# DeJhon-Huang/TrueTrace-Unity-Pathtracer

Hardware: AMD Instinct MI355X
Metric: Mrays/sec (primary+1-bounce) on Sponza CWBVH at 1080p; % HBM roofline (higher is better)
Workload: dtype f32

## Files before the change

### truetrace-unity-pathtracer_amd/csrc/tt_trace.hip

```cpp
#include "tt_launch.h"
#include "tt_wide.h"

#ifndef TT_LEAF_REFILL_MIN
#define TT_LEAF_REFILL_MIN (TT_LEAF_POOL ? 16 : TT_REFILL_MIN)
#endif

namespace {
template <int INFO, int LEAF = 0>
__device__ __forceinline__ bool write_record(const TraceArgs& A, uint32_t ray_index, uint32_t pix, float col_w,
                                             const Best& best, const LaneRay& wr, int32_t inst_mesh = 0,
                                             int32_t inst_tri_offset = 0) {
    tt_ray_data* R = A.rays + ray_index;
    const int32_t best_mesh = LEAF ? (best.tri_id != -1 ? inst_mesh : 0) : best.mesh_id;
    auto tri_offset_of_best = [&]() -> int32_t {
        if (LEAF) return best.tri_id != -1 ? inst_tri_offset : A.mesh[0].TriOffset;
        return A.mesh[best.mesh_id].TriOffset;
    };
    if (INFO != 0) {
        if (pix < A.n_pixels) {
            uint4 o;
            bool write = false;
            if (INFO == 1) {
                const int32_t to = tri_offset_of_best();
                o = make_uint4((uint32_t)best_mesh, (uint32_t)(best.tri_id - to),
                               __float_as_uint(best.u), __float_as_uint(best.v));
                write = true;
            } else {
                const float w = col_w;
                if (w == -1.0f || (float)A.bounce == w) {
                    write = true;
                    const bool miss = best.t == A.far_plane;
                    if ((A.flags & TT_TRACE_USE_RESTIRGI) && !miss) {
                        const int32_t to = tri_offset_of_best();
                        o.x = (uint32_t)best_mesh;
                        o.y = (uint32_t)(best.tri_id - to);
                        o.z = (uint32_t)(best.u * 65535.0f) | ((uint32_t)(best.v * 65535.0f) << 16);
                    } else {
                        LaneRay w = wr;
                        if (LEAF == 1) {
                            const uint4* rp = reinterpret_cast<const uint4*>(R);
                            const uint4 r0 = rp[0], r1 = rp[1];
                            w.ox = __uint_as_float(r0.x);
                            w.oy = __uint_as_float(r0.y);
                            w.oz = __uint_as_float(r0.z);
                            w.dx = __uint_as_float(r1.x);
                            w.dy = __uint_as_float(r1.y);
                            w.dz = __uint_as_float(r1.z);
                        }
                        if ((A.flags & TT_TRACE_USE_ASVGF) || !miss) {
                            o.x = __float_as_uint(w.dx);
                            o.y = __float_as_uint(w.dy);
                            o.z = __float_as_uint(w.dz);
                        } else {
                            o.x = __float_as_uint(w.dx * best.t + w.ox);
                            o.y = __float_as_uint(w.dy * best.t + w.oy);
                            o.z = __float_as_uint(w.dz * best.t + w.oz);
                        }
                    }
                    o.w = miss ? 1u : 0u;
                }
            }
            if (write) reinterpret_cast<uint4*>(A.info)[pix] = o;
        }
    }
    const uint32_t uv = (uint32_t)(best.u * 65535.0f) | ((uint32_t)(best.v * 65535.0f) << 16);
    const uint4 hit = make_uint4((uint32_t)best_mesh, (uint32_t)best.tri_id, __float_as_uint(best.t), uv);
    reinterpret_cast<uint4*>(R)[2] = hit;
    if (A.hits_out) {
        const u32x4 v = {hit.x, hit.y, hit.z, hit.w};
        __builtin_amdgcn_raw_buffer_store_b128(v, buffer_rsrc(A.hits_out, 0x7fffffff), (ray_index - A.ray_offset) << 4,
                                               0, 0);
    }
    return best.t != A.far_plane;
}

__device__ __forceinline__ void keep_record(const TraceArgs& A, uint32_t ray_index) {
    if (A.hits_out) {
        const uint4 h = reinterpret_cast<const uint4*>(A.rays + ray_index)[2];
        const u32x4 v = {h.x, h.y, h.z, h.w};
        __builtin_amdgcn_raw_buffer_store_b128(v, buffer_rsrc(A.hits_out, 0x7fffffff), (ray_index - A.ray_offset) << 4,
                                               0, 0);
    }
}

static_assert(TT_CHUNK_BIG == 64, "the adaptive order maps one dequeue (TT_CHUNK_BIG rays) to one 64-ray chunk");
#ifndef TT_ORDER_MIN_REPS
#define TT_ORDER_MIN_REPS 32
#endif
__device__ __forceinline__ void record_chunk_cost(const TraceArgs& A, bool swizzle, uint32_t ray_index, int32_t reps) {
    if (reps < TT_ORDER_MIN_REPS) return;
    const uint32_t local = ray_index - A.ray_offset;
    uint32_t c = local >> 6;
    if (swizzle) {
        const uint32_t py = fastdiv(local, A.div_width), px = local - py * A.width;
        c = (py >> 3) * (A.width >> 3) + (px >> 3);
    }
    atomicMax(A.chunk_cost + c, (uint32_t)reps);
}
}


namespace {
__device__ __forceinline__ bool root_leaf_hit(const RootLeaf& R, const LaneRay& r, float max_distance) {
    const float adjx = __uint_as_float(rl_byte(R.e, 0) << 23) * r.ix;
    const float adjy = __uint_as_float(rl_byte(R.e, 1) << 23) * r.iy;
    const float adjz = __uint_as_float(rl_byte(R.e, 2) << 23) * r.iz;
    const float orgx = r.ix * (R.px - r.ox);
    const float orgy = r.iy * (R.py - r.oy);
    const float orgz = r.iz * (R.pz - r.oz);
    const bool nx = r.dx < 0.0f, ny = r.dy < 0.0f, nz = r.dz < 0.0f;
    const uint32_t x_min = rl_byte(nx ? R.qhi : R.qlo, 0), x_max = rl_byte(nx ? R.qlo : R.qhi, 0);
    const uint32_t y_min = rl_byte(ny ? R.qhi : R.qlo, 1), y_max = rl_byte(ny ? R.qlo : R.qhi, 1);
    const uint32_t z_min = rl_byte(nz ? R.qhi : R.qlo, 2), z_max = rl_byte(nz ? R.qlo : R.qhi, 2);
    const float tminx = fma_((float)x_min, adjx, orgx);
    const float tminy = fma_((float)y_min, adjy, orgy);
    const float tminz = fma_((float)z_min, adjz, orgz);
    const float tmaxx = fma_((float)x_max, adjx, orgx);
    const float tmaxy = fma_((float)y_max, adjy, orgy);
    const float tmaxz = fma_((float)z_max, adjz, orgz);
    const float tmin = fmaxf(fmaxf(tminx, tminy), fmaxf(tminz, 1e-8f));
    float tmaxz_c;
    asm("v_min_f32 %0, %1, %2" : "=v"(tmaxz_c) : "v"(tmaxz), "v"(max_distance));
    const float tmax = fminf(fminf(tmaxx, tmaxy), tmaxz_c);
    return tmin < tmax;
}
}


template <bool STATS, bool MATCHECK, int INFO, bool IND, bool ORD, int LEAF = 0>
__device__ __forceinline__ void trace_body(const TraceArgs& A) {
    static_assert(!LEAF || (!STATS && !MATCHECK && !ORD), "the leaf-TLAS form has no stats / material / order variants");
    constexpr bool POOL = LEAF != 0 && TT_LEAF_POOL != 0;
    constexpr int tt_lds_depth = lds_depth_of<LEAF>();
    static_assert(!POOL || TT_CHUNK_BIG == TT_WAVE, "the prepared-ray pool holds one chunk, one slot per lane");
    __shared__ uint2 s_stack[tt_lds_depth][TT_BLOCK];
    __shared__ uint4 s_pool[POOL ? 3 : 1][TT_BLOCK];
    (void)s_pool;
    LeafEntry L{};
    if (LEAF) L = load_leaf_mesh<true>(A.leaf, A.root.base_tri + firstbithigh(A.root.bits));
    const uint32_t tid = threadIdx.x;
    zero_next_control(A.ctl_next, tid);
    const uint32_t gtid = blockIdx.x * TT_BLOCK + tid;
    const uint32_t spill_stride = gridDim.x * TT_BLOCK;
    uint2* __restrict__ spill = A.spill;
    (void)gtid;
    (void)spill_stride;
    (void)spill;
    const uint32_t lane = tid & (TT_WAVE - 1);
#ifdef TT_DIAG_BLOCKS
    if (tid < TT_DB_N) tt_db[tid] = 0ull;
    __syncthreads();
#endif

    uint32_t pool_next = 0, pool_end = 0, more = 1;
    const uint32_t wave_id = blockIdx.x * (TT_BLOCK / TT_WAVE) + (tid >> 6);
    SegState S{blockIdx.x % TT_SEGS, 0u, 0u};
    const uint32_t n_rays = IND ? launch_ray_count(A) : A.n_rays;
    const uint32_t n_tiles = (n_rays + 63u) >> 6;
    const bool swizzle = IND ? (A.tile_swizzle && n_rays == A.n_pixels) : (A.tile_swizzle != 0u);
    const __amdgpu_buffer_rsrc_t nodes = buffer_rsrc(A.nodes, A.n_nodes * (uint32_t)TT_NODE_STRIDE);
    const __amdgpu_buffer_rsrc_t tris = buffer_rsrc(A.tris, A.n_tris * (uint32_t)sizeof(TriPos));

    constexpr uint32_t TT_IDLE = 0x80000000u;
    uint32_t ray_index = 0;
    uint32_t pix = 0;
    float col_w = 0.0f;
    bool pending = false;
    LaneRay ray{}, wray{};
    Best best{};
    uint2 cg = make_uint2(0u, 0u), tg = make_uint2(0u, TT_IDLE);
    uint32_t oct = 0;
    int32_t stack_size = 0, tlas_ss = -1;
    int32_t NodeOffset = 0, TriOffset = 0, MatOffset = 0, mesh_id = -1, Reps = 0;
    if (LEAF) {
        NodeOffset = L.off.y;
        TriOffset = L.off.x;
        MatOffset = L.off.z;
        mesh_id = L.mesh_id;
    }
    uint32_t c_nodes = 0, c_tris = 0, c_blas = 0, c_acc = 0, c_rays = 0, c_hits = 0, c_reps = 0, c_ovf = 0;
    uint32_t d_iter = 0, d_node_lanes = 0, d_node_iters = 0, d_tri_lanes = 0, d_tri_iters = 0, d_active_lanes = 0;
    uint32_t d_lead_same = 0, d_uniform = 0;
    auto world_ray = [&]() -> LaneRay { return wray; };
    auto ray_of = [&](uint32_t widx) -> uint32_t {
        uint32_t local = widx;
        if (swizzle) {
            const uint32_t tw = A.width >> 3;
            const uint32_t t = widx >> 6, l = widx & 63u;
            const uint32_t ty = fastdiv(t, A.div_tiles), tx = t - ty * tw;
            local = (ty * 8u + (l >> 3)) * A.width + tx * 8u + (l & 7u);
        }
        return A.ray_offset + local;
    };
    (void)ray_of;

#if TT_ROOT_LEAF
    const bool rl_ok = A.root.ok != 0u;
#endif
    auto enter_blas = [&]() {
            TT_DB(8);
            const uint32_t mo = firstbithigh(tg.y);
            tg.y &= ~(1u << mo);
            const LeafEntry e = load_leaf_mesh<true>(A.leaf, tg.x + mo);
            mesh_id = e.mesh_id;
            NodeOffset = e.off.y;
            TriOffset = e.off.x;
            bool ok = true;
            if (tg.y != 0u) TT_PUSH(tg, ok);
            if (ok && (cg.y & 0xff000000u)) TT_PUSH(cg, ok);
            tg.y = 0u;
            if (ok) {
                tlas_ss = stack_size;
                MatOffset = e.off.z;
                enter_object_space(e, ray, oct, cg);
                if (STATS) c_blas++;
            } else {
                tg.y = TT_IDLE;
                if (STATS) c_ovf++;
                TT_REPORT_OVERFLOW(A);
                keep_record(A, ray_index);
            }
    };
    auto finish_ray = [&]() {
        const bool hit = write_record<INFO, LEAF>(A, ray_index, pix, col_w, best, world_ray(), mesh_id, TriOffset);
        if (STATS) c_hits += hit ? 1u : 0u;
        (void)hit;
        if (ORD) record_chunk_cost(A, swizzle, ray_index, Reps);
    };
    constexpr uint32_t REFILL_MIN = LEAF ? TT_LEAF_REFILL_MIN : TT_REFILL_MIN;
    while (true) {
        TT_DB(0);
        const uint64_t idle = __ballot((int32_t)tg.y < 0);
        const uint32_t n_idle = (uint32_t)__builtin_popcount((uint32_t)idle) + (uint32_t)__builtin_popcount((uint32_t)(idle >> 32));
        const bool pool_dry = !more && pool_next >= pool_end;
#if TT_DRAIN_PRIO
        if (pool_dry) __builtin_amdgcn_s_setprio(TT_DRAIN_PRIO);
#endif
        const bool to_wide = TT_WIDE && pool_dry && n_idle < TT_WAVE && TT_WAVE - n_idle <= TT_WIDE_ENTER;
        if ((n_idle == TT_WAVE && pool_dry) || (n_idle >= REFILL_MIN && !pool_dry) || to_wide) {
            if (pending) {
                TT_DB(1);
                finish_ray();
                pending = false;
            }
        }
        if (n_idle == TT_WAVE && pool_dry) break;
#if TT_WIDE
        if (to_wide) {
            TT_DB(13);
            WideState st{{ray, world_ray(), cg, tg, oct, stack_size, tlas_ss, NodeOffset, TriOffset, MatOffset, Reps,
                          ray_index, tid, gtid, (int32_t)tg.y >= 0},
                         best, mesh_id, pix, col_w};
            regroup<2, LEAF>(st, __ballot((int32_t)tg.y >= 0), lane);
            auto finish_wide = [&](const WideState& w) {
                const bool hit = write_record<INFO, LEAF>(A, w.ray_index, w.pix, w.col_w, w.best, w.wray, mesh_id, TriOffset);
                if (STATS) c_hits += hit ? 1u : 0u;
                if (ORD) record_chunk_cost(A, swizzle, w.ray_index, w.Reps);
            };
            auto exhaust_wide = [&](const WideState& w) {
                keep_record(A, w.ray_index);
                if (ORD) record_chunk_cost(A, swizzle, w.ray_index, w.Reps);
            };
            wide_phase<STATS, MATCHECK, 2, LEAF>(A, st, s_stack, spill, spill_stride, nodes, tris, lane,
                                           Counters{c_nodes, c_tris, c_blas, c_acc, c_hits, c_reps, c_ovf},
                                           finish_wide, exhaust_wide);
            break;
        }
#endif
        if (n_idle >= REFILL_MIN && !pool_dry) {
            TT_DB(2);
#if TT_LONG_PRIO
            if (__ballot((int32_t)tg.y >= 0 && Reps >= TT_LONG_PRIO) != 0ull) __builtin_amdgcn_s_setprio(TT_LONG_PRIO_LEVEL);
            else __builtin_amdgcn_s_setprio(0);
#endif
            const uint32_t avail = pool_end - pool_next;
            uint32_t new_base = 0, new_count = 0;
            if (avail < n_idle && more) {
                new_count = sched_reserve(A.ctl, n_rays, n_tiles, lane, n_idle - avail, wave_id, S, new_base);
                more = new_count > 0 ? 1u : 0u;
                if (ORD && A.order && new_count > 0)
                    new_base = (__builtin_amdgcn_readfirstlane(A.order[new_base >> 6]) << 6) | (new_base & 63u);
            }
            const PoolTake pt = pool_take<TT_UNIFORM_POOL != 0>(idle, n_idle, new_base, new_count, pool_next, pool_end, more);
            const uint32_t widx = pt.widx;
            pool_next = pt.pool_next;
            pool_end = pt.pool_end;
            more = pt.more;
            if constexpr (POOL) {
                const uint32_t pcol = tid - lane;
                const bool take = (int32_t)tg.y < 0 && widx != 0xffffffffu;
                const bool take_left = take && lane_prefix(idle) < min(avail, n_idle);
                uint4 p0 = make_uint4(0u, 0u, 0u, 0u), p1 = p0, p2 = p0;
                if (take_left) {
                    const uint32_t slot = pcol + (widx & 63u);
                    p0 = s_pool[0][slot];
                    p1 = s_pool[1][slot];
                    p2 = s_pool[2][slot];
                }
                __builtin_amdgcn_fence(__ATOMIC_ACQ_REL, "wavefront");
                __builtin_amdgcn_wave_barrier();
                if (new_count > 0) {
                    TT_DB(4);
                    uint4 q0 = make_uint4(0u, 0u, 0u, 0u), q1 = q0, q2 = q0;
                    if (lane < new_count) {
                        const uint4* rp = reinterpret_cast<const uint4*>(A.rays + ray_of(new_base + lane));
                        const uint4 r0 = rp[0], r1 = rp[1];
                        float cw = 0.0f;
                        if (INFO == 2) cw = (r0.w < A.n_pixels) ? A.colors[r0.w].Data[3] : 0.0f;
                        LaneRay r;
                        r.ox = __uint_as_float(r0.x);
                        r.oy = __uint_as_float(r0.y);
                        r.oz = __uint_as_float(r0.z);
                        r.dx = __uint_as_float(r1.x);
                        r.dy = __uint_as_float(r1.y);
                        r.dz = __uint_as_float(r1.z);
                        r.ix = rcp_rn(r.dx);
                        r.iy = rcp_rn(r.dy);
                        r.iz = rcp_rn(r.dz);
                        uint32_t o = 0u;
                        uint2 g = make_uint2(0u, 0u);
                        if (root_leaf_hit(A.root, r, A.far_plane)) enter_object_space(L, r, o, g);
                        q0 = make_uint4(__float_as_uint(r.ox), __float_as_uint(r.oy), __float_as_uint(r.oz),
                                        __float_as_uint(r.dx));
                        q1 = make_uint4(__float_as_uint(r.dy), __float_as_uint(r.dz), __float_as_uint(r.ix),
                                        __float_as_uint(r.iy));
                        q2 = make_uint4(__float_as_uint(r.iz), r0.w, __float_as_uint(cw), o | g.y);
                    }
                    s_pool[0][tid] = q0;
                    s_pool[1][tid] = q1;
                    s_pool[2][tid] = q2;
                }
                __builtin_amdgcn_fence(__ATOMIC_ACQ_REL, "wavefront");
                __builtin_amdgcn_wave_barrier();
                if (take && !take_left) {
                    const uint32_t slot = pcol + (widx & 63u);
                    p0 = s_pool[0][slot];
                    p1 = s_pool[1][slot];
                    p2 = s_pool[2][slot];
                }
                if (take) {
                    TT_DL(19, true);
                    ray_index = ray_of(widx);
                    ray.ox = __uint_as_float(p0.x);
                    ray.oy = __uint_as_float(p0.y);
                    ray.oz = __uint_as_float(p0.z);
                    ray.dx = __uint_as_float(p0.w);
                    ray.dy = __uint_as_float(p1.x);
                    ray.dz = __uint_as_float(p1.y);
                    ray.ix = __uint_as_float(p1.z);
                    ray.iy = __uint_as_float(p1.w);
                    ray.iz = __uint_as_float(p2.x);
                    pix = p2.y;
                    col_w = __uint_as_float(p2.z);
                    oct = p2.w & 0x7fffffffu;
                    cg = make_uint2((p2.w & 0x80000000u) ? (uint32_t)L.off.w : 0u, p2.w & 0x80000000u);
                    if (LEAF == 2) {
                        const uint4* rp = reinterpret_cast<const uint4*>(A.rays + ray_index);
                        const uint4 r0 = rp[0], r1 = rp[1];
                        wray.ox = __uint_as_float(r0.x);
                        wray.oy = __uint_as_float(r0.y);
                        wray.oz = __uint_as_float(r0.z);
                        wray.dx = __uint_as_float(r1.x);
                        wray.dy = __uint_as_float(r1.y);
                        wray.dz = __uint_as_float(r1.z);
                    }
                    best.t = A.far_plane;
                    best.u = 0.0f;
                    best.v = 0.0f;
                    best.mesh_id = 0;
                    best.tri_id = -1;
                    tg = make_uint2(0u, 0u);
                    stack_size = 0;
                    Reps = 1;
                }
            }
            if (!POOL && (int32_t)tg.y < 0 && widx != 0xffffffffu) {
                TT_DB(4);
                TT_DL(19, true);
                uint32_t local = widx;
                if (swizzle) {
                    const uint32_t tw = A.width >> 3;
                    const uint32_t t = widx >> 6, l = widx & 63u;
                    const uint32_t ty = fastdiv(t, A.div_tiles), tx = t - ty * tw;
                    local = (ty * 8u + (l >> 3)) * A.width + tx * 8u + (l & 7u);
                }
                ray_index = A.ray_offset + local;
                const uint4* rp = reinterpret_cast<const uint4*>(A.rays + ray_index);
                const uint4 r0 = rp[0], r1 = rp[1];
                pix = r0.w;
                if (INFO == 2) col_w = (pix < A.n_pixels) ? A.colors[pix].Data[3] : 0.0f;
                ray.ox = __uint_as_float(r0.x);
                ray.oy = __uint_as_float(r0.y);
                ray.oz = __uint_as_float(r0.z);
                ray.dx = __uint_as_float(r1.x);
                ray.dy = __uint_as_float(r1.y);
                ray.dz = __uint_as_float(r1.z);
                ray.ix = rcp_rn(ray.dx);
                ray.iy = rcp_rn(ray.dy);
                ray.iz = rcp_rn(ray.dz);
                best.t = A.far_plane;
                best.u = 0.0f;
                best.v = 0.0f;
                best.mesh_id = 0;
                best.tri_id = -1;
                tg = make_uint2(0u, 0u);
                stack_size = 0;
                if (LEAF) {
                    if (LEAF == 2) wray = ray;
                    cg = make_uint2(0u, 0u);
                    Reps = 1;
                    if (root_leaf_hit(A.root, ray, best.t)) enter_object_space(L, ray, oct, cg);
                }
                if (!LEAF) {
                    wray = ray;
                    oct = octant_inv4(ray);
                    cg = make_uint2(A.tlas_base, 0x80000000u);
                    tlas_ss = -1;
                    NodeOffset = (int32_t)A.tlas_base;
                    TriOffset = 0;
                    MatOffset = 0;
                    mesh_id = -1;
                    Reps = 0;
                }
                if (STATS) c_rays++;
#if TT_ROOT_LEAF
                if (!LEAF && rl_ok) {
                    const RootLeaf& RL = A.root;
                    const bool hit = root_leaf_hit(RL, ray, best.t);
                    cg = make_uint2(RL.base_child, 0u);
                    tg = make_uint2(RL.base_tri, hit ? RL.bits : 0u);
                    Reps = 1;
                    if (STATS) c_nodes++;
                    if (hit) enter_blas();
                }
#endif
            }
        }

        if (STATS) {
            const uint64_t nm = __ballot(tg.y == 0u && Reps < TT_MAX_REPS && (cg.y & 0xff000000u));
            const uint64_t am = __ballot((int32_t)tg.y >= 0);
            if (lane == 0) {
                d_iter++;
                d_node_lanes += (uint32_t)__popcll(nm);
                d_node_iters += nm ? 1u : 0u;
                d_active_lanes += (uint32_t)__popcll(am);
            }
        }
        if (tg.y == 0u) {
            TT_DB(5);
            if (Reps >= TT_MAX_REPS) {
                tg.y = TT_IDLE;
                if (STATS) c_reps++;
                keep_record(A, ray_index);
                if (ORD) record_chunk_cost(A, swizzle, ray_index, Reps);
            } else if (cg.y & 0xff000000u) {
                const uint32_t child = take_child(cg, oct);
                bool ok = true;
                if (cg.y & 0xff000000u) {
                    TT_DB(7);
                    TT_PUSH(cg, ok);
                }
                if (ok) {
                    TT_DB(6);
                    TT_DL(17, true);
                    if (STATS) {
                        const uint32_t lead = __builtin_amdgcn_readfirstlane(child);
                        const uint64_t same = __ballot(child == lead), all = __ballot(true);
                        d_lead_same += child == lead ? 1u : 0u;
                        d_uniform += (same == all && lane == (uint32_t)__builtin_ctzll(all)) ? 1u : 0u;
                    }
                    const NodeWords n = load_node<TT_NODE_CPOL>(nodes, child);
                    const uint32_t hitmask = node_intersect(n.n0, n.n1, n.n2, n.n3, n.n4, ray, oct, best.t);
                    cg = node_group(hitmask, n, NodeOffset);
                    tg = tri_group(hitmask, n, TriOffset);
                    Reps++;
                    if (STATS) c_nodes++;
                } else {
                    tg.y = TT_IDLE;
                    if (STATS) c_ovf++;
                    TT_REPORT_OVERFLOW(A);
                    keep_record(A, ray_index);
                }
            } else {
                tg = cg;
                cg = make_uint2(0u, 0u);
            }
            if (!LEAF && (int32_t)tg.y > 0 && tlas_ss == -1) enter_blas();
        }

        if (STATS) {
            const uint64_t tm = __ballot((int32_t)tg.y > 0);
            if (lane == 0) {
                d_tri_lanes += (uint32_t)__popcll(tm);
                d_tri_iters += tm ? 1u : 0u;
            }
        }
        if ((int32_t)tg.y > 0) {
            TT_DB(9);
            TT_DL(18, true);
            const uint32_t ti = firstbithigh(tg.y);
            tg.y &= ~(1u << ti);
            const bool acc = intersect_triangle<MATCHECK>(tris, A.mat, A.bounce == 0, A.flags, (int32_t)(tg.x + ti),
                                                          mesh_id, MatOffset, ray, best);
            if (STATS) {
                c_tris++;
                c_acc += acc ? 1u : 0u;
            }
        }

        if (tg.y == 0u && (cg.y & 0xff000000u) == 0u) {
            TT_DB(10);
            if (stack_size != 0) {
                TT_DB(11);
                if (!LEAF && stack_size == tlas_ss) {
                    TT_DB(12);
                    leave_blas(A.tlas_base, world_ray(), NodeOffset, TriOffset, tlas_ss, ray, oct);
                }
                TT_POP(cg);
            } else {
                pending = true;
                tg.y = TT_IDLE;
            }
        }
    }

#ifdef TT_DIAG_BLOCKS
    __syncthreads();
    if (tid < TT_DB_N && A.diag_times && tt_db[tid]) atomicAdd(A.diag_times + tid, tt_db[tid]);
#endif
    if (STATS) {
        const uint32_t v[8] = {wave_sum(c_rays), wave_sum(c_nodes), wave_sum(c_tris), wave_sum(c_blas),
                               wave_sum(c_hits), wave_sum(c_reps), wave_sum(c_ovf), wave_sum(c_acc)};
        if (lane == 0) {
#pragma unroll
            for (int k = 0; k < 8; k++)
                if (v[k]) atomicAdd(&A.ctl->stats[k], (unsigned long long)v[k]);
            const uint32_t d[6] = {d_iter, d_node_iters, d_node_lanes, d_tri_iters, d_tri_lanes, d_active_lanes};
#pragma unroll
            for (int k = 0; k < 6; k++) atomicAdd(&A.ctl->diag[k], (unsigned long long)d[k]);
        }
        const uint32_t ls = wave_sum(d_lead_same), un = wave_sum(d_uniform);
        if (lane == 0) {
            atomicAdd(&A.ctl->diag[6], (unsigned long long)ls);
            atomicAdd(&A.ctl->diag[7], (unsigned long long)un);
        }
    }
}

template <bool STATS, bool MATCHECK, int INFO>
__global__ TT_BOUNDS void tt_trace_kernel(TraceArgs A) {
    trace_body<STATS, MATCHECK, INFO, false, false>(A);
}
template <bool MATCHECK, int INFO>
__global__ TT_BOUNDS void tt_trace_kernel_indirect(TraceArgs A) {
    trace_body<false, MATCHECK, INFO, true, false>(A);
}
template <int INFO>
__global__ __launch_bounds__(TT_BLOCK) __attribute__((amdgpu_waves_per_eu(5))) void tt_trace_kernel_ord(TraceArgs A) {
    trace_body<false, false, INFO, false, true>(A);
}
template <int INFO>
__global__ TT_BOUNDS void tt_trace_kernel_ord_mat(TraceArgs A) {
    trace_body<false, true, INFO, false, true>(A);
}
#ifndef TT_LEAF_WAVES
#define TT_LEAF_WAVES(INFO) 6
#endif
#define TT_LEAF_BOUNDS __launch_bounds__(TT_BLOCK) __attribute__((amdgpu_waves_per_eu(TT_LEAF_WAVES(INFO))))
#ifndef TT_LEAF_WRAY_RESIDENT
#define TT_LEAF_WRAY_RESIDENT 1
#endif
#define TT_LEAF_FORM(INFO) ((INFO) == 2 && TT_LEAF_WRAY_RESIDENT ? 2 : 1)
template <bool IND, int INFO>
__global__ TT_LEAF_BOUNDS void tt_trace_leaf_kernel(TraceArgs A) {
    trace_body<false, false, INFO, IND, false, TT_LEAF_FORM(INFO)>(A);
}

template <bool S, bool M, int I>
static hipError_t launch_one(const TraceArgs& a, bool leaf, uint32_t grid, hipStream_t st) {
    if constexpr (!S && !M) {
        if (leaf) {
            if (a.n_rays_dev) hipLaunchKernelGGL((tt_trace_leaf_kernel<true, I>), dim3(grid), dim3(TT_BLOCK), 0, st, a);
            else hipLaunchKernelGGL((tt_trace_leaf_kernel<false, I>), dim3(grid), dim3(TT_BLOCK), 0, st, a);
            return hipGetLastError();
        }
    }
    if constexpr (!S) {
        if (a.n_rays_dev) {
            hipLaunchKernelGGL((tt_trace_kernel_indirect<M, I>), dim3(grid), dim3(TT_BLOCK), 0, st, a);
            return hipGetLastError();
        }
        if (a.chunk_cost) {
            if (M) hipLaunchKernelGGL((tt_trace_kernel_ord_mat<I>), dim3(grid), dim3(TT_BLOCK), 0, st, a);
            else hipLaunchKernelGGL((tt_trace_kernel_ord<I>), dim3(grid), dim3(TT_BLOCK), 0, st, a);
            return hipGetLastError();
        }
    }
    hipLaunchKernelGGL((tt_trace_kernel<S, M, I>), dim3(grid), dim3(TT_BLOCK), 0, st, a);
    return hipGetLastError();
}

template <bool S, bool M>
static hipError_t launch_info(const TraceArgs& a, int info, bool leaf, uint32_t grid, hipStream_t st) {
    if (info == 0) return launch_one<S, M, 0>(a, leaf, grid, st);
    if (info == 1) return launch_one<S, M, 1>(a, leaf, grid, st);
    return launch_one<S, M, 2>(a, leaf, grid, st);
}

hipError_t tt_launch_trace(const TraceArgs& a, bool stats, bool matcheck, int info, bool leaf, uint32_t grid,
                           hipStream_t st) {
    if (leaf && (stats || matcheck || a.chunk_cost || !root_one_instance(a.root))) return hipErrorInvalidValue;
    if (stats)
        return matcheck ? launch_info<true, true>(a, info, false, grid, st) : launch_info<true, false>(a, info, false, grid, st);
    return matcheck ? launch_info<false, true>(a, info, false, grid, st) : launch_info<false, false>(a, info, leaf, grid, st);
}

hipError_t tt_trace_occupancy_table(int* out24) {
    out24[0] = occupancy_of(tt_trace_kernel<false, false, 0>);
    out24[1] = occupancy_of(tt_trace_kernel<false, false, 1>);
    out24[2] = occupancy_of(tt_trace_kernel<false, false, 2>);
    out24[3] = occupancy_of(tt_trace_kernel<false, true, 0>);
    out24[4] = occupancy_of(tt_trace_kernel<false, true, 1>);
    out24[5] = occupancy_of(tt_trace_kernel<false, true, 2>);
    out24[6] = occupancy_of(tt_trace_kernel<true, false, 0>);
    out24[7] = occupancy_of(tt_trace_kernel<true, false, 1>);
    out24[8] = occupancy_of(tt_trace_kernel<true, false, 2>);
    out24[9] = occupancy_of(tt_trace_kernel<true, true, 0>);
    out24[10] = occupancy_of(tt_trace_kernel<true, true, 1>);
    out24[11] = occupancy_of(tt_trace_kernel<true, true, 2>);
    out24[12] = occupancy_of(tt_trace_kernel_ord<0>);
    out24[13] = occupancy_of(tt_trace_kernel_ord<1>);
    out24[14] = occupancy_of(tt_trace_kernel_ord<2>);
    out24[15] = occupancy_of(tt_trace_kernel_ord_mat<0>);
    out24[16] = occupancy_of(tt_trace_kernel_ord_mat<1>);
    out24[17] = occupancy_of(tt_trace_kernel_ord_mat<2>);
    out24[18] = occupancy_of(tt_trace_leaf_kernel<false, 0>);
    out24[19] = occupancy_of(tt_trace_leaf_kernel<false, 1>);
    out24[20] = occupancy_of(tt_trace_leaf_kernel<false, 2>);
    out24[21] = occupancy_of(tt_trace_leaf_kernel<true, 0>);
    out24[22] = occupancy_of(tt_trace_leaf_kernel<true, 1>);
    out24[23] = occupancy_of(tt_trace_leaf_kernel<true, 2>);
    return hipGetLastError();
}

uint32_t tt_trace_block_size() { return TT_BLOCK; }
uint32_t tt_trace_chunk_rays() { return TT_CHUNK_BIG; }
uint32_t tt_trace_lds_bytes(bool leaf) {
    const uint32_t stack = (uint32_t)((leaf ? lds_depth_of<1>() : lds_depth_of<0>()) * TT_BLOCK * sizeof(uint2));
    return stack + (leaf && TT_LEAF_POOL ? (uint32_t)(3 * TT_BLOCK * sizeof(uint4)) : 0u);
}
uint32_t tt_trace_spill_entries() {
    constexpr int depth = lds_depth_of<1>() < lds_depth_of<0>() ? lds_depth_of<1>() : lds_depth_of<0>();
    return depth >= TT_STACK_SIZE ? 0u : (uint32_t)(TT_STACK_SIZE - depth);
}
```

### truetrace-unity-pathtracer_amd/csrc/tt_traverse.h

```cpp
#ifndef TT_TRAVERSE_H
#define TT_TRAVERSE_H
#include "tt_device.h"

#define TT_WAVE 64
#ifndef TT_BLOCK
#define TT_BLOCK 64
#endif
#ifndef TT_SEGS
#define TT_SEGS 8
#endif
#ifndef TT_CHUNK_BIG
#define TT_CHUNK_BIG 64
#endif
#ifndef TT_REFILL_MIN
#define TT_REFILL_MIN 20
#endif
#ifndef TT_PUSH_FAST
#define TT_PUSH_FAST 1
#endif
#ifndef TT_DRAIN_PRIO
#define TT_DRAIN_PRIO 2
#endif
#ifndef TT_LONG_PRIO
#define TT_LONG_PRIO 64
#endif
#ifndef TT_LONG_PRIO_LEVEL
#define TT_LONG_PRIO_LEVEL 2
#endif
#ifndef TT_UNIFORM_POOL
#define TT_UNIFORM_POOL 1
#endif
#ifndef TT_LDS_STACK
#define TT_LDS_STACK 12
#endif
#ifndef TT_LEAF_POOL
#define TT_LEAF_POOL 1
#endif
#ifndef TT_LEAF_LDS_STACK
#define TT_LEAF_LDS_STACK 6
#endif
#ifndef TT_WAVES_PER_EU
#define TT_WAVES_PER_EU 0
#endif
#if TT_WAVES_PER_EU > 0
#define TT_BOUNDS __launch_bounds__(TT_BLOCK, TT_WAVES_PER_EU)
#else
#define TT_BOUNDS __launch_bounds__(TT_BLOCK)
#endif

#ifdef TT_DIAG_BLOCKS
#define TT_DB_N 32
__shared__ unsigned long long tt_db[TT_DB_N];
#define TT_DB(k)                                                                               \
    do {                                                                                       \
        const uint64_t m_ = __ballot(1);                                                       \
        if ((threadIdx.x & 63u) == (uint32_t)__builtin_ctzll(m_)) atomicAdd(&tt_db[k], 1ull); \
    } while (0)
#define TT_DL(k, pred)                                                                         \
    do {                                                                                       \
        const uint64_t p_ = __ballot(pred), m_ = __ballot(1);                                  \
        if ((threadIdx.x & 63u) == (uint32_t)__builtin_ctzll(m_))                              \
            atomicAdd(&tt_db[k], (unsigned long long)__popcll(p_));                            \
    } while (0)
#else
#define TT_DB(k) \
    do {         \
    } while (0)
#define TT_DL(k, pred) \
    do {               \
    } while (0)
#endif

namespace {

struct LaneRay {
    float ox, oy, oz, dx, dy, dz, ix, iy, iz;
};

__device__ __forceinline__ float fma_(float a, float b, float c) { return __builtin_fmaf(a, b, c); }
__device__ __forceinline__ uint32_t firstbithigh(uint32_t x) { return 31u - (uint32_t)__builtin_clz(x); }

__device__ __forceinline__ uint32_t octant_inv4(const LaneRay& r) {
    return (r.dx < 0.0f ? 0u : 0x04040404u) | (r.dy < 0.0f ? 0u : 0x02020202u) |
           (r.dz < 0.0f ? 0u : 0x01010101u);
}


typedef uint32_t u32x4 __attribute__((ext_vector_type(4)));
__device__ __forceinline__ __amdgpu_buffer_rsrc_t buffer_rsrc(const void* base, uint32_t bytes) {
    return __builtin_amdgcn_make_buffer_rsrc(const_cast<void*>(base), 0, (int)bytes, 0x00020000);
}
#ifndef TT_TRI_CPOL
#define TT_TRI_CPOL 0
#endif
#ifndef TT_NODE_CPOL
#define TT_NODE_CPOL 0
#endif
template <int CPOL = 0>
__device__ __forceinline__ uint4 buffer_load16(__amdgpu_buffer_rsrc_t r, uint32_t off) {
    const u32x4 v = __builtin_amdgcn_raw_buffer_load_b128(r, off, 0, CPOL);
    return make_uint4(v.x, v.y, v.z, v.w);
}
typedef uint32_t u32x2 __attribute__((ext_vector_type(2)));
template <int CPOL = 0>
__device__ __forceinline__ uint2 buffer_load8(__amdgpu_buffer_rsrc_t r, uint32_t off) {
    const u32x2 v = __builtin_amdgcn_raw_buffer_load_b64(r, off, 0, CPOL);
    return make_uint2(v.x, v.y);
}
template <int CPOL = 0>
__device__ __forceinline__ uint32_t buffer_load4(__amdgpu_buffer_rsrc_t r, uint32_t off) {
    return __builtin_amdgcn_raw_buffer_load_b32(r, off, 0, CPOL);
}
static_assert(TT_NODE_STRIDE == 80 || TT_NODE_STRIDE == 128, "node stride: 80 (the reference array) or 128");
__device__ __forceinline__ uint32_t node_offset(uint32_t i) {
    if (TT_NODE_STRIDE == 128) return i << 7;
    uint32_t r;
    asm("v_lshl_add_u32 %0, %1, 2, %1\n\tv_lshlrev_b32 %0, 4, %0" : "=&v"(r) : "v"(i));
    return r;
}
__device__ __forceinline__ uint32_t tri_offset(uint32_t i) {
    uint32_t r;
    asm("v_lshl_add_u32 %0, %1, 1, %1\n\tv_lshlrev_b32 %0, 4, %0" : "=&v"(r) : "v"(i));
    return r;
}

__device__ __forceinline__ uint32_t node_intersect(const uint4 n0, const uint4 n1, const uint4 n2,
                                                   const uint4 n3, const uint4 n4, const LaneRay& r,
                                                   uint32_t oct_inv4, float max_distance) {
    const uint32_t w = n0.w;
    uint32_t ex, ey, ez;
    asm("v_lshlrev_b32_sdwa %0, %1, %2 dst_sel:DWORD dst_unused:UNUSED_PAD src0_sel:DWORD src1_sel:BYTE_0"
        : "=v"(ex) : "s"(23u), "v"(w));
    asm("v_lshlrev_b32_sdwa %0, %1, %2 dst_sel:DWORD dst_unused:UNUSED_PAD src0_sel:DWORD src1_sel:BYTE_1"
        : "=v"(ey) : "s"(23u), "v"(w));
    asm("v_lshlrev_b32_sdwa %0, %1, %2 dst_sel:DWORD dst_unused:UNUSED_PAD src0_sel:DWORD src1_sel:BYTE_2"
        : "=v"(ez) : "s"(23u), "v"(w));
    const float adjx = __uint_as_float(ex) * r.ix;
    const float adjy = __uint_as_float(ey) * r.iy;
    const float adjz = __uint_as_float(ez) * r.iz;
    const float orgx = r.ix * (__uint_as_float(n0.x) - r.ox);
    const float orgy = r.iy * (__uint_as_float(n0.y) - r.oy);
    const float orgz = r.iz * (__uint_as_float(n0.z) - r.oz);
    const bool nx = r.dx < 0.0f, ny = r.dy < 0.0f, nz = r.dz < 0.0f;
    uint32_t hit_mask = 0;
#pragma unroll
    for (int i = 0; i < 2; i++) {
        const uint32_t meta4 = i == 0 ? n1.z : n1.w;
        const uint32_t is_inner4 = (meta4 & (meta4 << 1)) & 0x10101010u;
        const uint32_t inner_mask4 = (is_inner4 >> 1) - (is_inner4 >> 4);
        const uint32_t bit_index4 = (meta4 ^ (oct_inv4 & inner_mask4)) & 0x1f1f1f1fu;
        const uint32_t child_bits4 = (meta4 >> 5) & 0x07070707u;
        const uint32_t qlx = i == 0 ? n2.x : n2.y, qhx = i == 0 ? n2.z : n2.w;
        const uint32_t qly = i == 0 ? n3.x : n3.y, qhy = i == 0 ? n3.z : n3.w;
        const uint32_t qlz = i == 0 ? n4.x : n4.y, qhz = i == 0 ? n4.z : n4.w;
        const uint32_t x_min = nx ? qhx : qlx, x_max = nx ? qlx : qhx;
        const uint32_t y_min = ny ? qhy : qly, y_max = ny ? qly : qhy;
        const uint32_t z_min = nz ? qhz : qlz, z_max = nz ? qlz : qhz;
#pragma unroll
        for (int j = 0; j < 4; j++) {
            const float tminx = fma_((float)((x_min >> (j * 8)) & 0xffu), adjx, orgx);
            const float tminy = fma_((float)((y_min >> (j * 8)) & 0xffu), adjy, orgy);
            const float tminz = fma_((float)((z_min >> (j * 8)) & 0xffu), adjz, orgz);
            const float tmaxx = fma_((float)((x_max >> (j * 8)) & 0xffu), adjx, orgx);
            const float tmaxy = fma_((float)((y_max >> (j * 8)) & 0xffu), adjy, orgy);
            const float tmaxz = fma_((float)((z_max >> (j * 8)) & 0xffu), adjz, orgz);
            const float tmin = fmaxf(fmaxf(tminx, tminy), fmaxf(tminz, 1e-8f));
            float tmaxz_c;
            asm("v_min_f32 %0, %1, %2" : "=v"(tmaxz_c) : "v"(tmaxz), "v"(max_distance));
            const float tmax = fminf(fminf(tmaxx, tmaxy), tmaxz_c);
            uint32_t bits;
            if (j == 0)
                asm("v_lshlrev_b32_sdwa %0, %1, %2 dst_sel:DWORD dst_unused:UNUSED_PAD src0_sel:BYTE_0 src1_sel:BYTE_0"
                    : "=v"(bits) : "v"(bit_index4), "v"(child_bits4));
            else if (j == 1)
                asm("v_lshlrev_b32_sdwa %0, %1, %2 dst_sel:DWORD dst_unused:UNUSED_PAD src0_sel:BYTE_1 src1_sel:BYTE_1"
                    : "=v"(bits) : "v"(bit_index4), "v"(child_bits4));
            else if (j == 2)
                asm("v_lshlrev_b32_sdwa %0, %1, %2 dst_sel:DWORD dst_unused:UNUSED_PAD src0_sel:BYTE_2 src1_sel:BYTE_2"
                    : "=v"(bits) : "v"(bit_index4), "v"(child_bits4));
            else
                asm("v_lshlrev_b32_sdwa %0, %1, %2 dst_sel:DWORD dst_unused:UNUSED_PAD src0_sel:BYTE_3 src1_sel:BYTE_3"
                    : "=v"(bits) : "v"(bit_index4), "v"(child_bits4));
            hit_mask |= (tmin < tmax) ? bits : 0u;
        }
    }
    return hit_mask;
}


__device__ __forceinline__ uint32_t take_child(uint2& cg, uint32_t oct) {
    const uint32_t cio = firstbithigh(cg.y);
    const uint32_t slot = (cio - 24u) ^ (oct & 0xffu);
    const uint32_t rel = __builtin_popcount(cg.y & ~(0xffffffffu << slot));
    const uint32_t child = cg.x + rel;
    cg.y &= ~(1u << cio);
    return child;
}
struct NodeWords {
    uint4 n0, n1, n2, n3, n4;
};
template <int CPOL>
__device__ __forceinline__ NodeWords load_node(__amdgpu_buffer_rsrc_t nodes, uint32_t child) {
    const uint32_t no = node_offset(child);
    return NodeWords{buffer_load16<CPOL>(nodes, no), buffer_load16<CPOL>(nodes, no + 16u),
                     buffer_load16<CPOL>(nodes, no + 32u), buffer_load16<CPOL>(nodes, no + 48u),
                     buffer_load16<CPOL>(nodes, no + 64u)};
}
__device__ __forceinline__ uint2 node_group(uint32_t hitmask, const NodeWords& n, int32_t NodeOffset) {
    return make_uint2(n.n1.x + (uint32_t)NodeOffset, (hitmask & 0xff000000u) | (n.n0.w >> 24));
}
__device__ __forceinline__ uint2 tri_group(uint32_t hitmask, const NodeWords& n, int32_t TriOffset) {
    return make_uint2(n.n1.y + (uint32_t)TriOffset, hitmask & 0x00ffffffu);
}

struct LeafEntry {
    float4 m0, m1, m2;
    int4 off;
    int32_t mesh_id;
};
template <bool MESH_ID>
__device__ __forceinline__ LeafEntry load_leaf_mesh(const LeafMesh* leaf, uint32_t i) {
    const float4* mp = reinterpret_cast<const float4*>(leaf + i);
    LeafEntry e;
    e.m0 = mp[0];
    e.m1 = mp[1];
    e.m2 = mp[2];
    e.off = reinterpret_cast<const int4*>(mp)[3];
    e.mesh_id = MESH_ID ? reinterpret_cast<const int4*>(mp)[4].x : 0;
    return e;
}
__device__ __forceinline__ LaneRay to_object_space(const float4 m0, const float4 m1, const float4 m2, const LaneRay& ray) {
    LaneRay nr;
    nr.dx = fma_(m0.z, ray.dz, fma_(m0.y, ray.dy, m0.x * ray.dx));
    nr.dy = fma_(m1.z, ray.dz, fma_(m1.y, ray.dy, m1.x * ray.dx));
    nr.dz = fma_(m2.z, ray.dz, fma_(m2.y, ray.dy, m2.x * ray.dx));
    nr.ox = fma_(m0.z, ray.oz, fma_(m0.y, ray.oy, m0.x * ray.ox)) + m0.w;
    nr.oy = fma_(m1.z, ray.oz, fma_(m1.y, ray.oy, m1.x * ray.ox)) + m1.w;
    nr.oz = fma_(m2.z, ray.oz, fma_(m2.y, ray.oy, m2.x * ray.ox)) + m2.w;
    nr.ix = rcp_rn(nr.dx);
    nr.iy = rcp_rn(nr.dy);
    nr.iz = rcp_rn(nr.dz);
    return nr;
}
__device__ __forceinline__ void enter_object_space(const LeafEntry& e, LaneRay& ray, uint32_t& oct, uint2& cg) {
    ray = to_object_space(e.m0, e.m1, e.m2, ray);
    oct = octant_inv4(ray);
    cg = make_uint2((uint32_t)e.off.w, 0x80000000u);
}
__device__ __forceinline__ void leave_blas(uint32_t tlas_base, const LaneRay& wray, int32_t& NodeOffset,
                                           int32_t& TriOffset, int32_t& tlas_ss, LaneRay& ray, uint32_t& oct) {
    NodeOffset = (int32_t)tlas_base;
    TriOffset = 0;
    tlas_ss = -1;
    ray = wray;
    oct = octant_inv4(ray);
}

struct Best {
    float t, u, v;
    int32_t mesh_id, tri_id;
};

__device__ __forceinline__ float2 align_uv(float bu, float bv, const int32_t* tex, const float* scale) {
    if (tex[0] <= 0) return make_float2(-1.0f, -1.0f);
    const float dx = (float)(((uint32_t)tex[0]) & 0x7FFFu) / 16384.0f;
    const float dy = (float)(((uint32_t)tex[0]) >> 15) / 16384.0f;
    const float dz = (float)(((uint32_t)tex[1]) & 0x7FFFu) / 16384.0f;
    const float dw = (float)(((uint32_t)tex[1]) >> 15) / 16384.0f;
    float x = bu * scale[0] + scale[2];
    float y = bv * scale[1] + scale[3];
    x = x < 0.0f ? 1.0f - fmodf(fabsf(x), 1.0f) : fmodf(fabsf(x), 1.0f);
    y = y < 0.0f ? 1.0f - fmodf(fabsf(y), 1.0f) : fmodf(fabsf(y), 1.0f);
    return make_float2(x * (dx - dz) + dz, y * (dy - dw) + dw);
}
__device__ __forceinline__ float2 align_uv(float2 b, const CutoutMat& m) { return align_uv(b.x, b.y, m.alpha_tex, m.scale); }
__device__ __forceinline__ int atlas_clamp(float c, uint32_t n) { return (int)fminf(fmaxf(c, 0.0f), (float)(n - 1u)); }
__device__ __forceinline__ float atlas_texel(const MatView& M, int x, int y) {
    return (float)M.atlas[(size_t)y * M.atlas_w + (size_t)x] / 255.0f;
}
__device__ __forceinline__ float sample_point(const MatView& M, float2 uv) {
    return atlas_texel(M, atlas_clamp(floorf(uv.x * (float)M.atlas_w), M.atlas_w),
                       atlas_clamp(floorf(uv.y * (float)M.atlas_h), M.atlas_h));
}
__device__ __forceinline__ float sample_linear(const MatView& M, float2 uv) {
    const float x = uv.x * (float)M.atlas_w - 0.5f, y = uv.y * (float)M.atlas_h - 0.5f;
    const float x0 = floorf(x), y0 = floorf(y);
    const float fx = x - x0, fy = y - y0;
    const int ix0 = atlas_clamp(x0, M.atlas_w), ix1 = atlas_clamp(x0 + 1.0f, M.atlas_w);
    const int iy0 = atlas_clamp(y0, M.atlas_h), iy1 = atlas_clamp(y0 + 1.0f, M.atlas_h);
    const float a = atlas_texel(M, ix0, iy0) * (1.0f - fx) + atlas_texel(M, ix1, iy0) * fx;
    const float b = atlas_texel(M, ix0, iy1) * (1.0f - fx) + atlas_texel(M, ix1, iy1) * fx;
    return a * (1.0f - fy) + b * fy;
}
__device__ __forceinline__ float half_bits_to_float(uint32_t h) {
    return (float)__builtin_bit_cast(_Float16, (uint16_t)h);
}
__device__ __forceinline__ float3 sample_tex_point(const MatView& M, float2 uv) {
    const int x = atlas_clamp(floorf(uv.x * (float)M.tex_w), M.tex_w);
    const int y = atlas_clamp(floorf(uv.y * (float)M.tex_h), M.tex_h);
    const uint2 t = M.tex[(size_t)y * M.tex_w + (size_t)x];
    return make_float3(half_bits_to_float(t.x & 0xffffu), half_bits_to_float(t.x >> 16),
                       half_bits_to_float(t.y & 0xffffu));
}
__device__ __forceinline__ float3 glass_tint(const MatView& M, const GlassMat& g, float2 buv) {
    const float3 x = sample_tex_point(M, align_uv(buv.x, buv.y, g.albedo_tex, g.scale));
    return make_float3((g.color[0] * (x.x + 2.0f)) / 3.0f, (g.color[1] * (x.y + 2.0f)) / 3.0f,
                       (g.color[2] * (x.z + 2.0f)) / 3.0f);
}

__device__ __forceinline__ float2 base_uv(const MatView& M, int32_t tri_id, float u, float v) {
    const float2* t = reinterpret_cast<const float2*>(reinterpret_cast<const char*>(M.raw + tri_id) + 60);
    const float2 t0 = t[0], t1 = t[1], t2 = t[2];
    const float w = 1.0f - u - v;
    return make_float2(t0.x * w + t1.x * u + t2.x * v, t0.y * w + t1.y * u + t2.y * v);
}

struct TriCand {
    float t, u, v;
    bool cand, accept;
};
struct TriData {
    uint4 a, b;
    uint2 c;
};
template <bool MATCHECK, int CPOL = TT_TRI_CPOL>
__device__ __forceinline__ TriData triangle_load(__amdgpu_buffer_rsrc_t tris, int32_t tri_id) {
    const uint32_t to = tri_offset((uint32_t)tri_id);
    TriData d;
    d.a = buffer_load16<CPOL>(tris, to);
    d.b = buffer_load16<CPOL>(tris, to + 16u);
    if (MATCHECK) {
        d.c = buffer_load8<CPOL>(tris, to + 32u);
    } else {
        d.c.x = buffer_load4<CPOL>(tris, to + 32u);
        d.c.y = 0u;
    }
    return d;
}
struct TriHit {
    float t, u, v;
};
#define TT_IN_TRIANGLE(u, v) (((u) >= 0.0f) && ((v) >= 0.0f && (u) + (v) <= 1.0f))
__device__ __forceinline__ TriHit triangle_hit(const TriData& d, const LaneRay& r) {
    const uint4 a = d.a, b = d.b;
    const float p0x = __uint_as_float(a.x), p0y = __uint_as_float(a.y), p0z = __uint_as_float(a.z);
    const float e1x = __uint_as_float(a.w), e1y = __uint_as_float(b.x), e1z = __uint_as_float(b.y);
    const float e2x = __uint_as_float(b.z), e2y = __uint_as_float(b.w), e2z = __uint_as_float(d.c.x);
    const float hx = fma_(r.dy, e2z, -(r.dz * e2y));
    const float hy = fma_(r.dz, e2x, -(r.dx * e2z));
    const float hz = fma_(r.dx, e2y, -(r.dy * e2x));
    const float aa = fma_(e1z, hz, fma_(e1y, hy, e1x * hx));
    const float f = rcp_rn(aa);
    const float sx = r.ox - p0x, sy = r.oy - p0y, sz = r.oz - p0z;
    const float u = f * fma_(sz, hz, fma_(sy, hy, sx * hx));
    const float qx = fma_(sy, e1z, -(sz * e1y));
    const float qy = fma_(sz, e1x, -(sx * e1z));
    const float qz = fma_(sx, e1y, -(sy * e1x));
    const float v = f * fma_(r.dz, qz, fma_(r.dy, qy, r.dx * qx));
    const float t = f * fma_(e2z, qz, fma_(e2y, qy, e2x * qx));
    return TriHit{t, u, v};
}
__device__ __forceinline__ float3 normalize_pinned(float x, float y, float z) {
    const float inv = 1.0f / sqrtf(fma_(z, z, fma_(y, y, x * x)));
    return make_float3(x * inv, y * inv, z * inv);
}
__device__ __forceinline__ bool backfacing(float e1x, float e1y, float e1z, float e2x, float e2y, float e2z,
                                           const LaneRay& r) {
    const float3 a = normalize_pinned(e1x, e1y, e1z), b = normalize_pinned(e2x, e2y, e2z);
    const float3 n = normalize_pinned(fma_(a.y, b.z, -(a.z * b.y)), fma_(a.z, b.x, -(a.x * b.z)),
                                      fma_(a.x, b.y, -(a.y * b.x)));
    return fma_(n.z, r.dz, fma_(n.y, r.dy, n.x * r.dx)) <= 0.0f;
}

template <bool MATCHECK>
__device__ __forceinline__ TriCand triangle_test(const TriData& d, const MatView& M, bool bounce0, uint32_t tflags,
                                                 int32_t tri_id, int32_t mat_offset, const LaneRay& r, float best_t) {
    const TriHit h = triangle_hit(d, r);
    const float t = h.t, u = h.u, v = h.v;
    TriCand R;
    R.t = t;
    R.u = u;
    R.v = v;
    R.cand = TT_IN_TRIANGLE(u, v) && (t > 0.0f && t < best_t);
    R.accept = R.cand;
    if (MATCHECK && R.accept) {
        const uint32_t mi = (uint32_t)(mat_offset + (int32_t)d.c.y);
        const uint32_t w = mi < M.n_mat ? M.word[mi] : 0u;
        if ((w >> TT_MATWORD_CUTOUT) & 1u) {
            const CutoutMat cm = M.cut[mi];
            if (sample_linear(M, align_uv(base_uv(M, tri_id, u, v), cm)) < cm.cutoff) R.accept = false;
        }
        const bool glass = (w >> TT_MATWORD_GLASS) & 1u;
        if ((tflags & TT_TRACE_IGNORE_GLASS) && glass) R.accept = false;
        if ((tflags & TT_TRACE_IGNORE_BACKFACING) && bounce0 && !glass && R.accept &&
            backfacing(__uint_as_float(d.a.w), __uint_as_float(d.b.x), __uint_as_float(d.b.y), __uint_as_float(d.b.z),
                       __uint_as_float(d.b.w), __uint_as_float(d.c.x), r))
            R.accept = false;
        if (bounce0 && ((w >> TT_FLAG_INVISIBLE) & 1u)) R.accept = false;
    }
    return R;
}
template <bool MATCHECK>
__device__ __forceinline__ TriCand triangle_candidate(__amdgpu_buffer_rsrc_t tris, const MatView& M, bool bounce0,
                                                      uint32_t tflags, int32_t tri_id, int32_t mat_offset,
                                                      const LaneRay& r, float best_t) {
    return triangle_test<MATCHECK>(triangle_load<MATCHECK>(tris, tri_id), M, bounce0, tflags, tri_id, mat_offset, r,
                                   best_t);
}

template <bool MATCHECK>
__device__ __forceinline__ bool intersect_triangle(__amdgpu_buffer_rsrc_t tris, const MatView& M, bool bounce0, uint32_t tflags,
                                                   int32_t tri_id, int32_t mesh_id, int32_t mat_offset,
                                                   const LaneRay& r, Best& best) {
    const TriCand c = triangle_candidate<MATCHECK>(tris, M, bounce0, tflags, tri_id, mat_offset, r, best.t);
    if (c.accept) {
        best.t = c.t;
        best.u = c.u;
        best.v = c.v;
        best.mesh_id = mesh_id;
        best.tri_id = tri_id;
    }
    return c.cand;
}

__device__ __forceinline__ uint32_t seg_lo(uint32_t n_tiles, uint32_t seg) {
    return (uint32_t)(((uint64_t)n_tiles * seg / TT_SEGS) << 6);
}
struct SegState {
    uint32_t seg;
    uint32_t dead;
    uint32_t est;
};
__device__ __forceinline__ uint32_t sched_reserve(TraceControl* ctl, uint32_t n_rays, uint32_t n_tiles, uint32_t lane,
                                                  uint32_t need, uint32_t wave_id, SegState& S, uint32_t& base) {
    while (S.dead != (1u << TT_SEGS) - 1u) {
        const uint32_t lo = seg_lo(n_tiles, S.seg);
        const uint32_t hi = min(seg_lo(n_tiles, S.seg + 1), n_rays);
        const uint32_t len = hi > lo ? hi - lo : 0u;
        const uint32_t want = max(need, (uint32_t)TT_CHUNK_BIG);
        uint32_t off = 0;
        TT_DB(3);
        if (lane == 0) off = atomicAdd(&ctl->seg_ticket[S.seg * 32u], want);
        off = __builtin_amdgcn_readfirstlane(off);
        if (off < len) {
            S.est = off + want;
            base = lo + off;
            return min(want, len - off);
        }
        S.dead |= 1u << S.seg;
        const uint32_t start = (S.seg + 1u + wave_id % (TT_SEGS - 1u)) % TT_SEGS;
#pragma unroll
        for (uint32_t k = 0; k < TT_SEGS; k++) {
            const uint32_t c = (start + k) % TT_SEGS;
            if (!((S.dead >> c) & 1u)) {
                S.seg = c;
                break;
            }
        }
        S.est = 0;
    }
    return 0u;
}

__device__ __forceinline__ uint32_t lane_prefix(uint64_t mask) {
    return __builtin_amdgcn_mbcnt_hi((uint32_t)(mask >> 32), __builtin_amdgcn_mbcnt_lo((uint32_t)mask, 0u));
}

struct PoolTake {
    uint32_t widx, pool_next, pool_end, more;
};
template <bool UNIFORM>
__device__ __forceinline__ PoolTake pool_take(uint64_t idle, uint32_t n_idle, uint32_t new_base, uint32_t new_count,
                                              uint32_t pool_next, uint32_t pool_end, uint32_t more) {
    const uint32_t avail = pool_end - pool_next;
    const uint32_t take_old = min(avail, n_idle);
    const uint32_t take_new = min(n_idle - take_old, new_count);
    const uint32_t rank = lane_prefix(idle);
    uint32_t widx = 0xffffffffu;
    if (rank < take_old) widx = pool_next + rank;
    else if (rank - take_old < take_new) widx = new_base + (rank - take_old);
    if (new_count > 0) {
        pool_next = new_base + take_new;
        pool_end = new_base + new_count;
    } else {
        pool_next += take_old;
    }
    if (UNIFORM) {
        pool_next = __builtin_amdgcn_readfirstlane(pool_next);
        pool_end = __builtin_amdgcn_readfirstlane(pool_end);
        more = __builtin_amdgcn_readfirstlane(more);
    }
    return PoolTake{widx, pool_next, pool_end, more};
}

__device__ __forceinline__ void zero_next_control(TraceControl* next, uint32_t tid) {
    if (blockIdx.x == 0 && next) {
        uint32_t* w = reinterpret_cast<uint32_t*>(next);
        for (uint32_t i = tid; i < (uint32_t)(sizeof(TraceControl) / 4); i += TT_BLOCK) w[i] = 0u;
    }
}

__device__ __forceinline__ uint32_t wave_sum(uint32_t v) {
#pragma unroll
    for (int off = 32; off > 0; off >>= 1) v += __shfl_xor(v, off, TT_WAVE);
    return v;
}

template <class Kernel>
int occupancy_of(Kernel kernel) {
    int b = 0;
// ... 54 lines not shown
```

Measured before the change: 7297.

## Pre-intersect BLAS root node during ray pool refill using scalar-loaded root

When the leaf-TLAS prepared-ray pool is refilled, the single mesh's BLAS root node is loaded once per wave through scalar loads and intersected with each new ray. The resulting child hit mask is stored in the pool slot so traversal starts one level below the root. This drops the per-ray vector fetch and first traversal step of the root node. In exchange, refill does more work, the pool slot layout is repacked (col_w is folded into pix, oct is moved), and inline-asm scalar loads with a manual waitcnt are added.

```diff
diff --git a/truetrace-unity-pathtracer_amd/csrc/tt_trace.hip b/truetrace-unity-pathtracer_amd/csrc/tt_trace.hip
--- a/truetrace-unity-pathtracer_amd/csrc/tt_trace.hip
+++ b/truetrace-unity-pathtracer_amd/csrc/tt_trace.hip
@@ -131,6 +131,7 @@
 __device__ __forceinline__ void trace_body(const TraceArgs& A) {
     static_assert(!LEAF || (!STATS && !MATCHECK && !ORD), "the leaf-TLAS form has no stats / material / order variants");
     constexpr bool POOL = LEAF != 0 && TT_LEAF_POOL != 0;
+    constexpr bool ROOTSTEP = POOL && TT_LEAF_ROOT_STEP != 0;
     constexpr int tt_lds_depth = lds_depth_of<LEAF>();
     static_assert(!POOL || TT_CHUNK_BIG == TT_WAVE, "the prepared-ray pool holds one chunk, one slot per lane");
     __shared__ uint2 s_stack[tt_lds_depth][TT_BLOCK];
@@ -138,6 +139,13 @@
     (void)s_pool;
     LeafEntry L{};
     if (LEAF) L = load_leaf_mesh<true>(A.leaf, A.root.base_tri + firstbithigh(A.root.bits));
+    uint32_t root_cg_x = 0, root_tg_x = 0, root_imask = 0;
+    if (ROOTSTEP) {
+        const NodeWords n = load_node_uniform(A.nodes, A.n_nodes, (uint32_t)L.off.w);
+        root_cg_x = n.n1.x + (uint32_t)L.off.y;
+        root_tg_x = n.n1.y + (uint32_t)L.off.x;
+        root_imask = n.n0.w >> 24;
+    }
     const uint32_t tid = threadIdx.x;
     zero_next_control(A.ctl_next, tid);
     const uint32_t gtid = blockIdx.x * TT_BLOCK + tid;
@@ -290,18 +298,65 @@
                 const uint32_t pcol = tid - lane;
                 const bool take = (int32_t)tg.y < 0 && widx != 0xffffffffu;
                 const bool take_left = take && lane_prefix(idle) < min(avail, n_idle);
+                auto start_ray = [&](const uint4 p0, const uint4 p1, const uint4 p2) {
+                    TT_DL(19, true);
+                    ray_index = ray_of(widx);
+                    ray.ox = __uint_as_float(p0.x);
+                    ray.oy = __uint_as_float(p0.y);
+                    ray.oz = __uint_as_float(p0.z);
+                    ray.dx = __uint_as_float(p0.w);
+                    ray.dy = __uint_as_float(p1.x);
+                    ray.dz = __uint_as_float(p1.y);
+                    ray.ix = __uint_as_float(p1.z);
+                    ray.iy = __uint_as_float(p1.w);
+                    ray.iz = __uint_as_float(p2.x);
+                    pix = p2.y;
+                    if (ROOTSTEP) {
+                        col_w = -1.0f;
+                        oct = p2.z & 0x7fffffffu;
+                        const uint32_t inner = p2.w & 0xff000000u;
+                        cg = make_uint2(root_cg_x, inner ? (inner | root_imask) : 0u);
+                        tg = make_uint2(root_tg_x, p2.w & 0x00ffffffu);
+                        Reps = (p2.z & 0x80000000u) ? 2 : 1;
+                    } else {
+                        col_w = __uint_as_float(p2.z);
+                        oct = p2.w & 0x7fffffffu;
+                        cg = make_uint2((p2.w & 0x80000000u) ? (uint32_t)L.off.w : 0u, p2.w & 0x80000000u);
+                    }
+                    if (LEAF == 2) {
+                        const uint4* rp = reinterpret_cast<const uint4*>(A.rays + ray_index);
+                        const uint4 r0 = rp[0], r1 = rp[1];
+                        wray.ox = __uint_as_float(r0.x);
+                        wray.oy = __uint_as_float(r0.y);
+                        wray.oz = __uint_as_float(r0.z);
+                        wray.dx = __uint_as_float(r1.x);
+                        wray.dy = __uint_as_float(r1.y);
+                        wray.dz = __uint_as_float(r1.z);
+                    }
+                    best.t = A.far_plane;
+                    best.u = 0.0f;
+                    best.v = 0.0f;
+                    best.mesh_id = 0;
+                    best.tri_id = -1;
+                    if (!ROOTSTEP) tg = make_uint2(0u, 0u);
+                    stack_size = 0;
+                    if (!ROOTSTEP) Reps = 1;
+                };
                 uint4 p0 = make_uint4(0u, 0u, 0u, 0u), p1 = p0, p2 = p0;
                 if (take_left) {
                     const uint32_t slot = pcol + (widx & 63u);
                     p0 = s_pool[0][slot];
                     p1 = s_pool[1][slot];
                     p2 = s_pool[2][slot];
+                    if (ROOTSTEP) start_ray(p0, p1, p2);
                 }
                 __builtin_amdgcn_fence(__ATOMIC_ACQ_REL, "wavefront");
                 __builtin_amdgcn_wave_barrier();
                 if (new_count > 0) {
                     TT_DB(4);
                     uint4 q0 = make_uint4(0u, 0u, 0u, 0u), q1 = q0, q2 = q0;
+                    NodeWords rn{};
+                    if (ROOTSTEP) rn = load_node_uniform(A.nodes, A.n_nodes, (uint32_t)L.off.w);
                     if (lane < new_count) {
                         const uint4* rp = reinterpret_cast<const uint4*>(A.rays + ray_of(new_base + lane));
                         const uint4 r0 = rp[0], r1 = rp[1];
@@ -319,16 +374,32 @@
                         r.iz = rcp_rn(r.dz);
                         uint32_t o = 0u;
                         uint2 g = make_uint2(0u, 0u);
-                        if (root_leaf_hit(A.root, r, A.far_plane)) enter_object_space(L, r, o, g);
+                        const bool root_hit = root_leaf_hit(A.root, r, A.far_plane);
+                        TT_DL(29, root_hit);
+                        if (root_hit) enter_object_space(L, r, o, g);
                         q0 = make_uint4(__float_as_uint(r.ox), __float_as_uint(r.oy), __float_as_uint(r.oz),
                                         __float_as_uint(r.dx));
                         q1 = make_uint4(__float_as_uint(r.dy), __float_as_uint(r.dz), __float_as_uint(r.ix),
                                         __float_as_uint(r.iy));
                         q2 = make_uint4(__float_as_uint(r.iz), r0.w, __float_as_uint(cw), o | g.y);
+                        if (ROOTSTEP) {
+                            if (INFO == 2 && !(cw == -1.0f || (float)A.bounce == cw)) q2.y = 0xffffffffu;
+                            q2.z = o | g.y;
+                            q2.w = 0u;
+                            s_pool[0][tid] = q0;
+                            s_pool[1][tid] = q1;
+                            s_pool[2][tid] = q2;
+                            if (root_hit) {
+                                TT_DB(28);
+                                s_pool[2][tid].w = node_intersect(rn.n0, rn.n1, rn.n2, rn.n3, rn.n4, r, o, A.far_plane);
+                            }
+                        }
                     }
-                    s_pool[0][tid] = q0;
-                    s_pool[1][tid] = q1;
-                    s_pool[2][tid] = q2;
+                    if (!ROOTSTEP) {
+                        s_pool[0][tid] = q0;
+                        s_pool[1][tid] = q1;
+                        s_pool[2][tid] = q2;
+                    }
                 }
                 __builtin_amdgcn_fence(__ATOMIC_ACQ_REL, "wavefront");
                 __builtin_amdgcn_wave_barrier();
@@ -337,42 +408,9 @@
                     p0 = s_pool[0][slot];
                     p1 = s_pool[1][slot];
                     p2 = s_pool[2][slot];
-                }
-                if (take) {
-                    TT_DL(19, true);
-                    ray_index = ray_of(widx);
-                    ray.ox = __uint_as_float(p0.x);
-                    ray.oy = __uint_as_float(p0.y);
-                    ray.oz = __uint_as_float(p0.z);
-                    ray.dx = __uint_as_float(p0.w);
-                    ray.dy = __uint_as_float(p1.x);
-                    ray.dz = __uint_as_float(p1.y);
-                    ray.ix = __uint_as_float(p1.z);
-                    ray.iy = __uint_as_float(p1.w);
-                    ray.iz = __uint_as_float(p2.x);
-                    pix = p2.y;
-                    col_w = __uint_as_float(p2.z);
-                    oct = p2.w & 0x7fffffffu;
-                    cg = make_uint2((p2.w & 0x80000000u) ? (uint32_t)L.off.w : 0u, p2.w & 0x80000000u);
-                    if (LEAF == 2) {
-                        const uint4* rp = reinterpret_cast<const uint4*>(A.rays + ray_index);
-                        const uint4 r0 = rp[0], r1 = rp[1];
-                        wray.ox = __uint_as_float(r0.x);
-                        wray.oy = __uint_as_float(r0.y);
-                        wray.oz = __uint_as_float(r0.z);
-                        wray.dx = __uint_as_float(r1.x);
-                        wray.dy = __uint_as_float(r1.y);
-                        wray.dz = __uint_as_float(r1.z);
-                    }
-                    best.t = A.far_plane;
-                    best.u = 0.0f;
-                    best.v = 0.0f;
-                    best.mesh_id = 0;
-                    best.tri_id = -1;
-                    tg = make_uint2(0u, 0u);
-                    stack_size = 0;
-                    Reps = 1;
-                }
+                    if (ROOTSTEP) start_ray(p0, p1, p2);
+                }
+                if (!ROOTSTEP && take) start_ray(p0, p1, p2);
             }
             if (!POOL && (int32_t)tg.y < 0 && widx != 0xffffffffu) {
                 TT_DB(4);
diff --git a/truetrace-unity-pathtracer_amd/csrc/tt_traverse.h b/truetrace-unity-pathtracer_amd/csrc/tt_traverse.h
--- a/truetrace-unity-pathtracer_amd/csrc/tt_traverse.h
+++ b/truetrace-unity-pathtracer_amd/csrc/tt_traverse.h
@@ -38,6 +38,9 @@
 #endif
 #ifndef TT_LEAF_LDS_STACK
 #define TT_LEAF_LDS_STACK 6
+#endif
+#ifndef TT_LEAF_ROOT_STEP
+#define TT_LEAF_ROOT_STEP 1
 #endif
 #ifndef TT_WAVES_PER_EU
 #define TT_WAVES_PER_EU 0
@@ -206,6 +209,23 @@
                      buffer_load16<CPOL>(nodes, no + 32u), buffer_load16<CPOL>(nodes, no + 48u),
                      buffer_load16<CPOL>(nodes, no + 64u)};
 }
+__device__ __forceinline__ NodeWords load_node_uniform(const uint4* nodes, uint32_t n_nodes, uint32_t node) {
+    u32x4 a = {0u, 0u, 0u, 0u}, b = a, c = a, d = a, e = a;
+    if (node < n_nodes) {
+        const char* p = reinterpret_cast<const char*>(nodes) + (size_t)node * TT_NODE_STRIDE;
+        asm volatile("s_nop 4\n\t"
+                     "s_load_dwordx4 %0, %5, 0x0\n\t"
+                     "s_load_dwordx4 %1, %5, 0x10\n\t"
+                     "s_load_dwordx4 %2, %5, 0x20\n\t"
+                     "s_load_dwordx4 %3, %5, 0x30\n\t"
+                     "s_load_dwordx4 %4, %5, 0x40\n\t"
+                     "s_waitcnt lgkmcnt(0)"
+                     : "=&s"(a), "=&s"(b), "=&s"(c), "=&s"(d), "=&s"(e)
+                     : "s"(p));
+    }
+    return NodeWords{make_uint4(a.x, a.y, a.z, a.w), make_uint4(b.x, b.y, b.z, b.w), make_uint4(c.x, c.y, c.z, c.w),
+                     make_uint4(d.x, d.y, d.z, d.w), make_uint4(e.x, e.y, e.z, e.w)};
+}
 __device__ __forceinline__ uint2 node_group(uint32_t hitmask, const NodeWords& n, int32_t NodeOffset) {
     return make_uint2(n.n1.x + (uint32_t)NodeOffset, (hitmask & 0xff000000u) | (n.n0.w >> 24));
 }
```

Result: faster. 7522, median of 6 (+3.1%).
